# SungFeng-Huang/Meta-TTS

Hardware: AMD Instinct MI355X
Metric: meta-steps/sec (8-task meta-batch, 5 inner steps) (higher is better)
Workload: dtype f32; 1 GPU; C3: Meta-TTS MAML first-order (algorithm=meta_emb_vad, inner=5, meta-batch=8 tasks x (5 support + 5 query utts)), FastSpeech2 base.yaml, outer mean + clip(1.0) + Adam/Noam; meta_batch=8, tasks_per_gpu=8, inner_steps=5, order=first, parallelism=task-dp1, numerics=fp32 MFMA (v_mfma_f32_32x32x2_f32), dropout=on (0.2 / 0.5 / 0.5, counter-based masks), batch_ingestion=inside every timed step (host 12-tuples -> HBM + plans)

## Files before the change

include/mtts.h:

```cpp
#ifndef MTTS_H
#define MTTS_H

#include <stdint.h>

#ifdef __cplusplus
extern "C" {
#endif

typedef struct mtts_handle mtts_handle;

typedef struct mtts_model_cfg {
    int d_model, enc_layers, dec_layers, enc_heads, dec_heads, d_ff, k1, k2;
    int vp_filter, vp_kernel, n_bins, max_seq_len, n_mel, vocab, n_speaker;
    int postnet_dim, postnet_kernel, postnet_layers;
    float pitch_min, pitch_max, energy_min, energy_max;
    int adapt_mask;
    float enc_dropout, dec_dropout, vp_dropout;
    int pitch_frame_level, energy_frame_level;
} mtts_model_cfg;

typedef struct mtts_batch {
    int B, S_max, T_max;
    const int64_t* speakers;
    const int64_t* texts;
// ... 82 lines not shown
int mtts_profile_kinds(void);
const char* mtts_profile_kernel_name(int kind);
int mtts_profile_report(mtts_handle* h, double* out, int kinds);

int mtts_gemm_f32(int form, int M, int N, int K, const float* A, int lda, const float* B, int ldb, float* C, int ldc,
                  const float* bias, float alpha, int flags, int tile, void* hip_stream);
int mtts_gemm_f32_dual(int form, int M, int N, int K, const float* A, int lda, const float* B, int ldb, const float* A2, const float* B2,
                       float* C, int ldc, const float* bias, float alpha, int flags, int tile, void* hip_stream);
int mtts_gemm_bf16(int form, int M, int N, int K, const float* A, int lda, const float* B, int ldb, const float* A2, const float* B2,
                   float* C, int ldc, const float* bias, float alpha, int flags, int tile, void* hip_stream);
int mtts_to_bf16(const float* src, unsigned short* dst, long long n, void* stream);
int mtts_gemm_bf16_planes(int M, int N, int K, const unsigned short* Ah, int lda, const unsigned short* Bh, int ldb, float* C, unsigned short* Ch,
                          int ldc, const float* bias, float alpha, int flags, int tile, void* stream);
long long mtts_plane_problems(mtts_handle* h);
int mtts_xcd_schedule_check(const int* dims, int groups, int cls, int tn, int units_per_group, int* max_load_permille);
int mtts_conv1d_f32(int mode, int L, int Cin, int Cout, int k, const float* x_or_dy, const float* w_or_x, float* out,
                    const float* bias, int tile, void* hip_stream);

int64_t mtts_kernel_ws_bytes(int rows, int n_mat);
int mtts_layernorm_fwd(int rows, int C, const float* a, const float* res, const float* gamma, const float* beta, const unsigned char* mask,
                       float* z, float* y, float* stats, void* ws, void* hip_stream);
int mtts_layernorm_bwd(int rows, int C, const float* dy, const float* z, const float* stats, const float* gamma, const unsigned char* mask,
                       float* dz, float* dgamma, float* dbeta, void* ws, void* hip_stream);
int mtts_softmax_fwd(int n_mat, int L, float* S, void* ws, void* hip_stream);
int mtts_softmax_bwd(int n_mat, int L, const float* P, float* dP, float alpha, void* ws, void* hip_stream);
int mtts_sdpa_fwd(int n_mat, int L, int dk, const float* q, const float* k, const float* v, float* P, float* o, void* ws, void* hip_stream);
int mtts_batchnorm_fwd(int rows, int C, const float* x, const unsigned char* inrect, const float* gamma, const float* beta, int do_tanh,
                       float* stats, float* y, void* ws, void* hip_stream);
int mtts_batchnorm_bwd(int rows, int n_in, int C, const float* dy, const float* y, const float* x, const float* stats, const unsigned char* inrect,
                       const float* gamma, int do_tanh, float* dx, float* dgamma, float* dbeta, void* ws, void* hip_stream);
// ... 140 lines not shown
```

meta_tts_amd/_lib.py:

```python
from __future__ import annotations

import ctypes as C
import os

HERE = os.path.dirname(os.path.abspath(__file__))
DEFAULT_LIB = os.path.join(HERE, "libmtts.so")


class ModelCfg(C.Structure):
    _fields_ = [(n, C.c_int) for n in (
        "d_model", "enc_layers", "dec_layers", "enc_heads", "dec_heads", "d_ff", "k1", "k2",
        "vp_filter", "vp_kernel", "n_bins", "max_seq_len", "n_mel", "vocab", "n_speaker",
        "postnet_dim", "postnet_kernel", "postnet_layers")] + [
        ("pitch_min", C.c_float), ("pitch_max", C.c_float), ("energy_min", C.c_float), ("energy_max", C.c_float),
        ("adapt_mask", C.c_int), ("enc_dropout", C.c_float), ("dec_dropout", C.c_float), ("vp_dropout", C.c_float),
        ("pitch_frame_level", C.c_int), ("energy_frame_level", C.c_int)]


class Batch(C.Structure):
    _fields_ = [("B", C.c_int), ("S_max", C.c_int), ("T_max", C.c_int),
                ("speakers", C.c_void_p), ("texts", C.c_void_p), ("src_lens", C.c_void_p),
                ("mels", C.c_void_p), ("mel_lens", C.c_void_p), ("pitches", C.c_void_p),
                ("energies", C.c_void_p), ("durations", C.c_void_p), ("spk_emb", C.c_void_p)]

# ... 55 lines not shown
    "mtts_sync_pack": (C.c_int, [C.c_void_p, C.c_float]),
    "mtts_sync_unpack": (C.c_int, [C.c_void_p]),
    "mtts_get_synced_losses": (C.c_int, [C.c_void_p, C.c_void_p]),
    "mtts_set_bn_sync": (C.c_int, [C.c_void_p, C.c_int]),
    "mtts_outer_update": (C.c_int, [C.c_void_p, C.c_void_p, C.c_float, C.c_float, C.c_float, C.c_float, C.c_float,
                                    C.c_float, C.c_void_p]),
    "mtts_reset_optimizer": (C.c_int, [C.c_void_p]),
    "mtts_set_grad_accumulation": (C.c_int, [C.c_void_p, C.c_int]),
    "mtts_profile_gemm": (C.c_int, [C.c_void_p, C.c_int]),
    "mtts_profile_kinds": (C.c_int, []),
    "mtts_profile_kernel_name": (C.c_char_p, [C.c_int]),
    "mtts_profile_report": (C.c_int, [C.c_void_p, C.POINTER(C.c_double), C.c_int]),
    "mtts_gemm_f32": (C.c_int, [C.c_int, C.c_int, C.c_int, C.c_int, C.c_void_p, C.c_int, C.c_void_p, C.c_int, C.c_void_p,
                                C.c_int, C.c_void_p, C.c_float, C.c_int, C.c_int, C.c_void_p]),
    "mtts_xcd_schedule_check": (C.c_int, [C.POINTER(C.c_int), C.c_int, C.c_int, C.c_int, C.c_int, C.POINTER(C.c_int)]),
    "mtts_gemm_f32_dual": (C.c_int, [C.c_int, C.c_int, C.c_int, C.c_int, C.c_void_p, C.c_int, C.c_void_p, C.c_int, C.c_void_p, C.c_void_p,
                                     C.c_void_p, C.c_int, C.c_void_p, C.c_float, C.c_int, C.c_int, C.c_void_p]),
    "mtts_to_bf16": (C.c_int, [C.c_void_p, C.c_void_p, C.c_longlong, C.c_void_p]),
    "mtts_gemm_bf16_planes": (C.c_int, [C.c_int, C.c_int, C.c_int, C.c_void_p, C.c_int, C.c_void_p, C.c_int, C.c_void_p, C.c_void_p, C.c_int,
                                        C.c_void_p, C.c_float, C.c_int, C.c_int, C.c_void_p]),
    "mtts_plane_problems": (C.c_longlong, [C.c_void_p]),
    "mtts_gemm_bf16": (C.c_int, [C.c_int, C.c_int, C.c_int, C.c_int, C.c_void_p, C.c_int, C.c_void_p, C.c_int, C.c_void_p, C.c_void_p,
                                 C.c_void_p, C.c_int, C.c_void_p, C.c_float, C.c_int, C.c_int, C.c_void_p]),
    "mtts_conv1d_f32": (C.c_int, [C.c_int, C.c_int, C.c_int, C.c_int, C.c_int, C.c_void_p, C.c_void_p, C.c_void_p,
                                  C.c_void_p, C.c_int, C.c_void_p]),
    "mtts_kernel_ws_bytes": (C.c_int64, [C.c_int, C.c_int]),
    "mtts_layernorm_fwd": (C.c_int, [C.c_int, C.c_int] + [C.c_void_p] * 10),
    "mtts_layernorm_bwd": (C.c_int, [C.c_int, C.c_int] + [C.c_void_p] * 10),
    "mtts_softmax_fwd": (C.c_int, [C.c_int, C.c_int, C.c_void_p, C.c_void_p, C.c_void_p]),
    "mtts_softmax_bwd": (C.c_int, [C.c_int, C.c_int, C.c_void_p, C.c_void_p, C.c_float, C.c_void_p, C.c_void_p]),
# ... 123 lines not shown
```

meta_tts_amd/csrc/gemm.h:

```cpp
#pragma once
#include <algorithm>
#include <cmath>
#include <cstdio>
#include <cstdlib>
#include <vector>

#include "compat.h"
#include "devres.h"
#include "knobs.h"

namespace mtts {

enum GemmForm { GEMM_NT = 0, GEMM_NN = 1, GEMM_TN = 2,
                GEMM_NT_H = 3 };
enum GemmFlags { GEMM_RELU = 1, GEMM_ACCUM = 2, GEMM_LRELU = 4 };

struct GemmGroupDesc {
    long long a_off, b_off, c_off;
    int M, N, K;
    int lda, ldb, ldc;
};

struct XcdSched {
    int on = 0;
// ... 105 lines not shown
    long long colsum_gs = 0;
    const float* colsum_w = nullptr;
    long long colsum_w_gs = 0;
    const float* A2 = nullptr;
    const float* B2 = nullptr;
    long long a2_gs = 0, b2_gs = 0;
    const bf16_t* Ah = nullptr;
    const bf16_t* Bh = nullptr;
    long long bh_gs = 0;
    bf16_t* Ch = nullptr;
    bool plane_only = false;
    LnFuse ln;
    const int* host_dims = nullptr;
    XcdSched xs;
    int wave_prio = 0;
};
inline int gemm_keff(const GemmArgs& g) { return g.A2 ? 2 * g.K : g.K; }


__device__ __forceinline__ int xcd_group_size(int tiles_n, int splitk) {
    const int G = tiles_n * (splitk > 1 ? splitk : 1);
    return G < 64 ? G : 64;
}
__device__ __forceinline__ int xcd_group_remap(int lin, int total, int G) {
    if (G <= 1) return lin;
    const int run = 8 * G, blk = lin / run;
    if ((blk + 1) * run > total) return lin;
    const int r = lin - blk * run;
    return blk * run + (r & 7) * G + (r >> 3);
}
// ... 695 lines not shown
}

template <int BM, int BN, int BK, int KL = 0>
__global__ __launch_bounds__(256) void gemm_f32_multi_dual_kernel(GemmMulti mp) {
    constexpr int F0 = GemmSmem<GEMM_NT, BM, BN, BK>::FLOATS, F1 = GemmSmem<GEMM_NN, BM, BN, BK>::FLOATS, F2 = GemmSmem<GEMM_TN, BM, BN, BK>::FLOATS;
    constexpr int FL = F0 > F1 ? (F0 > F2 ? F0 : F2) : (F1 > F2 ? F1 : F2);
    __shared__ __attribute__((aligned(16))) float smem[FL];
    int p, z, bx;
    if (!gemm_multi_locate(mp, p, z, bx)) return;
    const int form = mp.form[p];
    if (form == GEMM_NT) gemm_f32_body<GEMM_NT, BM, BN, BK, true, 2, 2, 0, true, KL>(mp.g[p], z, bx, smem);
    else if (form == GEMM_NN) gemm_f32_body<GEMM_NN, BM, BN, BK, true, 2, 2, 0, true, KL>(mp.g[p], z, bx, smem);
    else gemm_f32_body<GEMM_TN, BM, BN, BK, true, 2, 2, 0, true, KL>(mp.g[p], z, bx, smem);
}

enum GemmKind {
    GK_F32_64_BK16 = 0,
    GK_F32_64_BK32 = 3,
    GK_F32_128 = 6,
    GK_GLDS = 9,
    GK_MULTI16 = 12, GK_MULTI32 = 13, GK_GLDS_MULTI = 14, GK_OTHER = 15,
    GK_MULTI16_DUAL = 16, GK_MULTI32_DUAL = 17, GK_GLDS_MULTI_DUAL = 18,
    GK_BF16_64 = 19,
    GK_BF16_128 = 22,
    GK_BF16_MULTI64 = 25, GK_BF16_MULTI128 = 26, GK_BF16_MULTI64_DUAL = 27, GK_BF16_MULTI128_DUAL = 28,
    GK_ATTN_FWD = 29,
    GK_BF16_64_H64 = 30, GK_BF16_64_H32 = 31, GK_BF16_128_H = 32,
    GK_BF16_MULTI64_PLANES = 33,
    GK_COUNT = 34
};
inline const char* gemm_kind_name(int k) {
    static const char* names[GK_COUNT] = {
        "gemm_f32_kernel<0, 64, 64, 16, true, 2, 2, 0, 4>", "gemm_f32_kernel<1, 64, 64, 16, true, 2, 2, 0, 4>", "gemm_f32_kernel<2, 64, 64, 16, true, 2, 2, 0, 4>",
        "gemm_f32_kernel<0, 64, 64, 32, true, 2, 2, 0, 4>", "gemm_f32_kernel<1, 64, 64, 32, true, 2, 2, 0, 4>", "gemm_f32_kernel<2, 64, 64, 32, true, 2, 2, 0, 4>",
        "gemm_f32_kernel<0, 128, 128, ...>", "gemm_f32_kernel<1, 128, 128, ...>", "gemm_f32_kernel<2, 128, 128, ...>",
        "gemm_glds_kernel<0>", "gemm_glds_kernel<1>", "gemm_glds_kernel<2>",
        "gemm_f32_multi_kernel<64, 64, 16, 4>", "gemm_f32_multi_kernel<64, 64, 32, 4>", "gemm_glds_multi_kernel",
        "gemm_f32_kernel<other>", "gemm_f32_multi_dual_kernel<64, 64, 16, 4>", "gemm_f32_multi_dual_kernel<64, 64, 32, 4>", "gemm_glds_multi_dual_kernel",
        "gemm_bf16_kernel<0, 64, 64, 32, 1>", "gemm_bf16_kernel<1, 64, 64, 32, 1>", "gemm_bf16_kernel<2, 64, 64, 32, 1>",
        "gemm_bf16_kernel<0, 128, 128, 32, 1>", "gemm_bf16_kernel<1, 128, 128, 32, 1>", "gemm_bf16_kernel<2, 128, 128, 32, 1>",
        "gemm_bf16_multi_kernel<64, 64, 32, 1, false>", "gemm_bf16_multi_kernel<128, 128, 32, 1, false>",
        "gemm_bf16_multi_kernel<64, 64, 32, 1, true>", "gemm_bf16_multi_kernel<128, 128, 32, 1, true>", "attn_fwd_kernel",
        "gemm_bf16_kernel<3, 64, 64, 64, 1>", "gemm_bf16_kernel<3, 64, 64, 32, 1>", "gemm_bf16_kernel<3, 128, 128, 32, 1>",
        "gemm_bf16_multi_planes_kernel<64, 64, 32, 64, 1>"};
    return (k >= 0 && k < GK_COUNT) ? names[k] : "?";
}

struct GemmProfiler {
    struct Rec { int kernel; double flops; hipEvent_t e0, e1; int form = 0, tile = 0, N = 0, K = 0, groups = 0, splitk = 1; double rows = 0, bytes = 0; int tag = 0; };
    int ctx = 0;
    int tag = 0;
    std::vector<Rec> recs;
    std::vector<hipEvent_t> pool;
    size_t used = 0;
    bool enabled = false;
    hipEvent_t get(DevHeap& heap) {
        if (used == pool.size()) { hipEvent_t e = nullptr; heap.event(e); pool.push_back(e); }
        return pool[used++];
    }
// ... 18 lines not shown
inline int gemm_kloop_variant() { return knobs().kloop; }
inline int gemm_kloop_for(const GemmArgs& g, int bk) {
    const bool ok = (g.taps <= 1 || g.tap_k % bk == 0) && (g.a_tap_k >= 0x40000000 || g.a_tap_k % bk == 0);
    return ok ? gemm_kloop_variant() : 0;
}
inline int gemm_xcd_swizzle() { return kGemmXcdSwizzle; }
inline int gemm_default_bk() { return kGemmDefaultBk; }
inline bool gemm_default_pipe() { return kGemmDefaultPipe; }

struct GemmWorkspace { float* ws = nullptr; int* ctr = nullptr; };
constexpr long long kSplitWsFloats = 16ll << 20;
constexpr int kSplitCtrs = 1 << 16;
constexpr int kLnCtrs = 4096;

struct GemmPending { int form; GemmArgs g; int max_M, max_N, groups; double flops, rows, bytes; };
struct GemmBatch { bool open = false; std::vector<GemmPending> q; int force_family = 0; int force_tile = 0; };

struct GemmCtx {
    GemmBatch batch;
    GemmProfiler prof;
    GemmWorkspace wsp;
    int last_kind = GK_OTHER;
    long long plane_problems = 0;
    bool bf16 = false;
    const char* error = nullptr;
    bool flushing = false;
    bool prefer_bk16 = false;
    int wave_prio = 0;
    bool no_glds = false;
    DevHeap* heap = nullptr;
    int alloc_workspace(DevHeap& h) {
// ... 31 lines not shown
inline bool gemm_use_glds() { return gemm_glds_mode() != 0; }
inline bool gemm_glds_ok(const GemmArgs& g) { return !(g.taps > 1 && g.tap_k % 32 != 0); }
inline int gemm_tiles_n(const GemmArgs& g, int max_N, int t) { return (max_N + t - 1) / t + (g.colsum ? 1 : 0); }
inline long gemm_glds_max_wgs() { return 768L; }
#if !defined(MTTS_EMU)
inline void gemm_glds_launch(int form, const GemmArgs& g, dim3 grid, hipStream_t stream);
inline void gemm_glds_multi_launch(const GemmMulti& mp, dim3 grid, hipStream_t stream, bool dual = false);
#endif

inline bool gemm_bf16_ok(const GemmArgs& g);
inline bool gemm_bf16_planes_ok(int form, const GemmArgs& g);
inline int gemm_bf16_launch(int form, const GemmArgs& g, int T, dim3 grid, hipStream_t stream, int pf);
inline int gemm_bf16_multi_launch(const GemmMulti& mp, int T, bool dual, dim3 grid, hipStream_t stream);
inline int gemm_bf16_tile(double rows, int tiles_n128) { return std::ceil(rows / 128.0) * tiles_n128 >= 512.0 ? 128 : 64; }

inline bool gemm_xcd_sched_for(GemmArgs& g, int max_M, int max_N, int groups, int S, int tile) {
    g.xs.on = 0;
    if (!knobs().xcd_sched || (groups != 8 && groups != 4 && groups != 2) || groups < knobs().xcd_sched_min_groups || !g.host_dims || !g.dimptr || g.table || S != 1) return false;
    int dims[8] = {0};
    for (int z = 0; z < groups; ++z) dims[z] = g.host_dims[z] * g.dim_mult;
    const int tn = gemm_tiles_n(g, max_N, tile);
    if (g.dim_sel == 0) xcd_sched_build(g.xs, dims, 1, tn, 0, tile, groups);
    else xcd_sched_build(g.xs, dims, 2, 1, ((max_M + tile - 1) / tile) * tn, 64, groups);
    if (g.xs.maxlen <= 0) g.xs.on = 0;
    if (knobs().xcd_sched_debug && g.xs.on) fprintf(stderr, "xcd_sched cls %d tn %d maxlen %d pool %d\n", g.xs.on, g.xs.tn, g.xs.maxlen, g.xs.P[8]);
    return g.xs.on != 0;
}
inline long gemm_xcd_sched_slots(const XcdSched& s) { return 8L * s.maxlen * (s.on == 1 ? s.tn : 1); }
inline bool gemm_panel_order_for(const GemmArgs& g, int form, double rows, int max_M, int max_N, int groups) {
    if (!knobs().panel_order || g.table || groups >= 8 || groups < 1) return false;
    if (std::ceil(rows / 64.0) * gemm_tiles_n(g, max_N, 64) > (double)gemm_glds_max_wgs()) return false;
    const double K = (double)gemm_keff(g);
    const double a_bytes = form == GEMM_TN ? rows * max_M : rows / groups * (g.lda > 0 ? g.lda : K);
    const double b_bytes = form == GEMM_TN ? rows * max_N : (double)max_N * K;
    (void)max_M;
    return b_bytes > a_bytes;
}

inline void gemm_launch(GemmCtx& cx, int form, const GemmArgs& g_in, int max_M, int max_N, int groups, hipStream_t stream,
                        int tile = 0, double alg_flops = 0.0, long long total_M = 0, double alg_bytes = 0.0) {
    if (max_M <= 0 || max_N <= 0 || groups <= 0) return;
    GemmArgs g = g_in;
    g.swizzle = gemm_xcd_swizzle();
    g.wave_prio = cx.wave_prio;
    if (!(cx.bf16 && gemm_bf16_ok(g) && gemm_bf16_planes_ok(form, g))) {
        if (g.plane_only) { cx.error = "plane-only GEMM problem outside the bf16 plane path"; return; }
        g.Ah = g.Bh = nullptr;
    }
    if (!cx.bf16) g.Ch = nullptr;
    const int user_tile = tile;
    const double rows = total_M > 0 ? (double)total_M : (double)max_M * groups;
// ... 24 lines not shown
    bool pipe = gemm_default_pipe();
    int bk = gemm_default_bk();
    bool glds = false;
    const bool bf16 = cx.bf16 && gemm_bf16_ok(g) && !g.A2;
    if (bf16 && user_tile == 0) tile = gemm_bf16_tile(rows, gemm_tiles_n(g, max_N, 128));
#if !defined(MTTS_EMU)
    if (bf16) { if (tile == 4064) tile = 64; }
    else if (tile == 4064) { glds = gemm_glds_ok(g); tile = 64; }
    else if (user_tile == 0 && tile == 64) {
        const long wgs = (long)std::ceil(rows / 64.0) * gemm_tiles_n(g, max_N, 64);
        glds = gemm_use_glds() && gemm_glds_ok(g) && wgs <= gemm_glds_max_wgs() && !cx.no_glds && !g.ln.y;
    }
#else
    if (tile == 4064) tile = 64;
#endif
    const int ablate = tile / 10000;
    tile %= 10000;
    if (tile >= 1000) { pipe = (tile / 1000) & 1; bk = (tile / 2000) ? 32 : 16; tile %= 1000; }
    if (user_tile == 0 && !g.table && gemm_keff(g) >= 1024 && (form == GEMM_NT || form == GEMM_TN)) bk = 32;
    if (g.taps > 1 && g.tap_k % 32 != 0) bk = 16;
    if (bf16) bk = 32;
    const int S = 1;
    { int used = 0; if (!gemm_ln_bind(cx, form, g, max_M, groups, bf16 ? 0 : tile, used)) return; }
    const int nth = 256;
    const long grid_tiles = ntiles(tile);
    dim3 block(nth), grid((unsigned)(grid_tiles * S), 1, (unsigned)groups);
    if (gemm_xcd_sched_for(g, max_M, max_N, groups, S, tile)) grid = dim3((unsigned)gemm_xcd_sched_slots(g.xs), 1, 1);
    else if (gemm_panel_order_for(g, form, rows, max_M, max_N, groups)) {
        g.swizzle = 2; g.po_tiles_m = (max_M + tile - 1) / tile;
        grid = dim3((unsigned)xcd_panel_slots(g.po_tiles_m, gemm_tiles_n(g, max_N, tile), S), 1, (unsigned)groups);
    }
    GemmProfiler& prof = cx.prof;
    hipEvent_t e0 = nullptr, e1 = nullptr;
    if (prof.enabled) { e0 = prof.get(*cx.heap); e1 = prof.get(*cx.heap); hipEventRecord(e0, stream); }
    int kind = GK_OTHER;
#define MTTS_GEMM_CASE(F, T)                                                                              \
    if (form == F && tile == T) {                                                                         \
        if (pipe && T == 64) {                                                                            \
            const int kl = gemm_kloop_for(g, bk);                                                         \
            if (F == GEMM_NT && g.ln.ctr) {       \
                if (bk == 32) MTTS_LAUNCH((gemm_f32_kernel<GEMM_NT, 64, 64, 32, true, 2, 2, 0, 4, true>), grid, block, stream, g);   \
                else MTTS_LAUNCH((gemm_f32_kernel<GEMM_NT, 64, 64, 16, true, 2, 2, 0, 4, true>), grid, block, stream, g);            \
// ... 12 lines not shown
        else if (bk == 32 && pipe) { MTTS_LAUNCH((gemm_f32_kernel<F, T, T, 32, true>), grid, block, stream, g); kind = (T == 64 ? GK_F32_64_BK32 : GK_F32_128) + F; }   \
        else if (bk == 32) { MTTS_LAUNCH((gemm_f32_kernel<F, T, T, 32, false>), grid, block, stream, g); kind = T == 64 ? GK_OTHER : GK_F32_128 + F; }     \
        else if (pipe) { MTTS_LAUNCH((gemm_f32_kernel<F, T, T, 16, true>), grid, block, stream, g); kind = (T == 64 ? GK_F32_64_BK16 : GK_F32_128) + F; }          \
        else { MTTS_LAUNCH((gemm_f32_kernel<F, T, T, 16, false>), grid, block, stream, g); kind = T == 64 ? GK_OTHER : GK_F32_128 + F; }                   \
    }
    if (bf16) {
        if (g.Ah) ++cx.plane_problems;
        kind = gemm_bf16_launch(form, g, tile, grid, stream, (user_tile % 10000) / 1000);
    } else
#if !defined(MTTS_EMU)
    if (glds) {
        gemm_glds_launch(form, g, grid, stream);
        kind = GK_GLDS + form;
    } else
#endif
    {
#if defined(MTTS_GEMM_ABLATION)
#define MTTS_ABL(A) if (ablate == A && form == GEMM_NT) { MTTS_LAUNCH((gemm_f32_kernel<GEMM_NT, 64, 64, 16, true, 2, 2, A>), grid, block, stream, g); return; }
        MTTS_ABL(1) MTTS_ABL(2) MTTS_ABL(3) MTTS_ABL(4) MTTS_ABL(7) MTTS_ABL(8) MTTS_ABL(15) MTTS_ABL(6) MTTS_ABL(14)
#undef MTTS_ABL
#else
        (void)ablate;
#endif
        MTTS_GEMM_CASE(GEMM_NT, 128) MTTS_GEMM_CASE(GEMM_NT, 64)
        MTTS_GEMM_CASE(GEMM_NN, 128) MTTS_GEMM_CASE(GEMM_NN, 64)
        MTTS_GEMM_CASE(GEMM_TN, 128) MTTS_GEMM_CASE(GEMM_TN, 64)
    }
#undef MTTS_GEMM_CASE
    cx.last_kind = kind;
    if (prof.enabled) {
        hipEventRecord(e1, stream);
        GemmProfiler::Rec rec{kind, alg_flops, e0, e1};
        rec.form = form; rec.tile = bf16 ? 16000 + tile : (glds ? 4064 : tile); rec.N = max_N; rec.K = gemm_keff(g); rec.groups = groups; rec.splitk = S;
        rec.rows = rows;
        rec.bytes = alg_bytes; rec.tag = prof.tag;
        prof.recs.push_back(rec);
    }
}

inline bool batch_full_regime(const std::vector<GemmPending>& q) {
    double wgs = 0.0;
    for (const GemmPending& p : q) wgs += std::ceil(p.rows / 64.0) * gemm_tiles_n(p.g, p.max_N, 64);
    return wgs > (double)gemm_glds_max_wgs();
}
inline void gemm_batch_end(GemmCtx& cx, hipStream_t stream) {
    GemmBatch& b = cx.batch;
    b.open = false;
    if (b.q.empty()) return;
// ... 80 lines not shown
        max_groups = std::max(max_groups, p.groups);
        flops += p.flops; rows += p.rows; bytes += p.bytes;
    }
    hipEvent_t e0 = nullptr, e1 = nullptr;
    if (prof.enabled) { e0 = prof.get(*cx.heap); e1 = prof.get(*cx.heap); hipEventRecord(e0, stream); }
    dim3 block(256), grid((unsigned)mp.start[mp.n], 1, 1);
    bool bk32 = true;
    int maxK = 0;
    for (int i = 0; i < mp.n; ++i) {
        if (mp.g[i].taps > 1 && mp.g[i].tap_k % 32 != 0) bk32 = false;
        maxK = std::max(maxK, gemm_keff(mp.g[i]));
    }
    bool glds = gemm_use_glds() && small_batch && !cx.no_glds && ln_used == 0;
    if (b.force_family) { glds = b.force_family == 4064; bk32 = bk32 && b.force_family == 32; if (bk32) maxK = std::max(maxK, 1024); }
    for (int i = 0; i < mp.n; ++i) glds = glds && gemm_glds_ok(mp.g[i]);
    int kind = GK_MULTI16;
    if (bf16) {
        for (int i = 0; i < mp.n; ++i) if (mp.g[i].Ah) ++cx.plane_problems;
        kind = gemm_bf16_multi_launch(mp, T, any_dual, grid, stream);
        glds = false;
    } else
#if !defined(MTTS_EMU)
    if (glds) { gemm_glds_multi_launch(mp, grid, stream, any_dual); kind = any_dual ? GK_GLDS_MULTI_DUAL : GK_GLDS_MULTI; }
    else
#endif
    if (bk32 && maxK >= 1024 && !cx.prefer_bk16) {
        int kl = gemm_kloop_variant();
        for (int i = 0; i < mp.n; ++i) kl = std::min(kl, gemm_kloop_for(mp.g[i], 32));
        if (any_dual) {
            if (kl == 4) MTTS_LAUNCH((gemm_f32_multi_dual_kernel<64, 64, 32, 4>), grid, block, stream, mp);
            else if (kl == 1) MTTS_LAUNCH((gemm_f32_multi_dual_kernel<64, 64, 32, 1>), grid, block, stream, mp);
            else MTTS_LAUNCH((gemm_f32_multi_dual_kernel<64, 64, 32, 0>), grid, block, stream, mp);
            kind = GK_MULTI32_DUAL;
        } else {
            if (ln_used > 0) MTTS_LAUNCH((gemm_f32_multi_kernel<64, 64, 32, 4, true>), grid, block, stream, mp);
            else if (kl == 4) MTTS_LAUNCH((gemm_f32_multi_kernel<64, 64, 32, 4>), grid, block, stream, mp);
            else if (kl == 1) MTTS_LAUNCH((gemm_f32_multi_kernel<64, 64, 32, 1>), grid, block, stream, mp);
            else MTTS_LAUNCH((gemm_f32_multi_kernel<64, 64, 32, 0>), grid, block, stream, mp);
            kind = GK_MULTI32;
        }
    } else {
// ... 1 lines not shown
        for (int i = 0; i < mp.n; ++i) kl = std::min(kl, gemm_kloop_for(mp.g[i], 16) == 4 ? 4 : 0);
        if (any_dual) {
            if (kl == 4) MTTS_LAUNCH((gemm_f32_multi_dual_kernel<64, 64, 16, 4>), grid, block, stream, mp);
            else MTTS_LAUNCH((gemm_f32_multi_dual_kernel<64, 64, 16, 0>), grid, block, stream, mp);
            kind = GK_MULTI16_DUAL;
        } else {
            if (ln_used > 0) MTTS_LAUNCH((gemm_f32_multi_kernel<64, 64, 16, 4, true>), grid, block, stream, mp);
            else if (kl == 4) MTTS_LAUNCH((gemm_f32_multi_kernel<64, 64, 16, 4>), grid, block, stream, mp);
            else MTTS_LAUNCH((gemm_f32_multi_kernel<64, 64, 16, 0>), grid, block, stream, mp);
        }
    }
    cx.last_kind = kind;
    if (prof.enabled) {
        hipEventRecord(e1, stream);
        GemmProfiler::Rec rec{kind, flops, e0, e1};
        rec.form = 3; rec.tile = bf16 ? 16000 + T : (glds ? 4064 : 64); rec.N = mp.n; rec.K = maxK; rec.groups = mp.start[mp.n]; rec.splitk = max_split; rec.rows = rows; rec.bytes = bytes; rec.tag = prof.tag;
        prof.recs.push_back(rec);
    }
    b.q.clear();
}

}
```

meta_tts_amd/csrc/knobs.h:

```cpp
#pragma once
#include <cstdlib>

namespace mtts {

struct Knobs {
    int kloop = 4;
    int glds = 0;
    int xcd_sched = 1;
    int xcd_sched_min_groups = 8;
    int xcd_sched_debug = 0;
    int panel_order = 1;
    int single_multi = 1;
    int batch_splitk = 1;
    int defer_wgrad = 1;
    int side_pred_all = 1;
    int pred_side = 1;
    int pred_early = 1;
    int pred_batch = 1;
    int enc_ahead = 1;
    int enc_ahead_all = 1;
    int enc_ahead_query = 1;
    int upd_overlap = 1;
    int ln_fold_side = 1;
    int side_bk16 = 1;
    int main_prio = 1;
    int fused_attn = 1;
    int attn_sort = 1;
    int ln_fuse = 0;
    int so_keep_act = 1;
    int so_keep_grad = 1;
    int so_defer_post = 1;
    int so_fuse_drop = 1;
    int so_ln_part = 1;
    int so_pred_side = 1;
    int so_table_side = 1;
    int ablate_ln = 0;
    int attn_diag_mask = 0;
};

inline Knobs read_knobs() {
    Knobs k;
    const struct { const char* name; int* v; } table[] = {
        {"MTTS_KLOOP", &k.kloop}, {"MTTS_GLDS", &k.glds}, {"MTTS_XCD_SCHED", &k.xcd_sched}, {"MTTS_XCD_SCHED_MIN_GROUPS", &k.xcd_sched_min_groups},
        {"MTTS_PANEL_ORDER", &k.panel_order}, {"MTTS_SINGLE_MULTI", &k.single_multi}, {"MTTS_BATCH_SPLITK", &k.batch_splitk},
        {"MTTS_DEFER_WGRAD", &k.defer_wgrad}, {"MTTS_SIDE_PRED_ALL", &k.side_pred_all}, {"MTTS_PRED_SIDE", &k.pred_side}, {"MTTS_PRED_EARLY", &k.pred_early},
        {"MTTS_PRED_BATCH", &k.pred_batch}, {"MTTS_ENC_AHEAD", &k.enc_ahead}, {"MTTS_ENC_AHEAD_ALL", &k.enc_ahead_all}, {"MTTS_ENC_AHEAD_QUERY", &k.enc_ahead_query},
        {"MTTS_UPD_OVERLAP", &k.upd_overlap}, {"MTTS_LN_FOLD_SIDE", &k.ln_fold_side}, {"MTTS_SIDE_BK16", &k.side_bk16}, {"MTTS_MAIN_PRIO", &k.main_prio},
        {"MTTS_FUSED_ATTN", &k.fused_attn}, {"MTTS_ATTN_SORT", &k.attn_sort}, {"MTTS_LN_FUSE", &k.ln_fuse}, {"MTTS_SO_KEEP_ACT", &k.so_keep_act},
        {"MTTS_SO_KEEP_GRAD", &k.so_keep_grad}, {"MTTS_SO_DEFER_POST", &k.so_defer_post}, {"MTTS_SO_FUSE_DROP", &k.so_fuse_drop}, {"MTTS_SO_LN_PART", &k.so_ln_part},
        {"MTTS_SO_PRED_SIDE", &k.so_pred_side}, {"MTTS_SO_TABLE_SIDE", &k.so_table_side},
#if defined(MTTS_ABLATE)
        {"MTTS_ABLATE_LN", &k.ablate_ln},
#endif
#if defined(MTTS_ATTN_DIAG)
        {"MTTS_ATTN_DIAG_MASK", &k.attn_diag_mask},
#endif
    };
    for (const auto& t : table)
        if (const char* e = getenv(t.name)) *t.v = atoi(e);
    if (k.kloop != 0 && k.kloop != 1 && k.kloop != 4) k.kloop = 4;
    k.glds = k.glds != 0;
    k.xcd_sched_debug = getenv("MTTS_XCD_SCHED_DEBUG") != nullptr;
    return k;
}
inline const Knobs& knobs() {
    static const Knobs k = read_knobs();
    return k;
}

}
```

meta_tts_amd/csrc/mtts.hip:

```cpp
#include "../../include/mtts.h"

#include "comm.h"
#include "engine.h"
#include "vocoder.h"
#include "dvector.h"
#include "melfront.h"
#include "griffin.h"
#include "preprocess.h"
#include "resample.h"
#include "pitch.h"
#include "vad.h"
#include "speakereval.h"
#include "tsne.h"
#include "dtw.h"

using namespace mtts;

static int copy_losses_impl(Engine& e, const float* dev, float* host, int n);
static int copy_losses(Engine& e, const float* dev, float* host, int n) { return copy_losses_impl(e, dev, host, n); }

struct mtts_handle {
    Engine eng;
    Comm comm;
    float* sup_losses_dev = nullptr;
// ... 464 lines not shown
        for (int k = 0; k < GK_COUNT; ++k) for (int j = 0; j < 4; ++j) out[k * 4 + j] += r[k][j];
    }
    return 0;
}

static GemmCtx& kernel_ctx() {
    static thread_local GemmCtx cx;
    return cx;
}
static int kernel_launch_rc() {
    GemmCtx& cx = kernel_ctx();
    if (cx.error) { cx.error = nullptr; (void)hipGetLastError(); return -1; }
    return hipGetLastError() == hipSuccess ? 0 : -1;
}
static bool tile_code_ok(int tile) {
    return tile == 0 || tile == 4064 || ((tile % 1000 == 64 || tile % 1000 == 128) && tile % 10000 < 4000);
}

int mtts_gemm_f32(int form, int M, int N, int K, const float* A, int lda, const float* B, int ldb, float* C, int ldc,
                  const float* bias, float alpha, int flags, int tile, void* stream) {
    if (form < 0 || form > 2 || !tile_code_ok(tile)) return -1;
    GemmArgs g;
    g.A = A; g.B = B; g.C = C; g.lda = lda; g.ldb = ldb; g.ldc = ldc; g.M = M; g.N = N; g.K = K;
    g.bias = bias; g.alpha = alpha; g.flags = flags & 0xff;
    if (flags & ~0xff) return -1;
    gemm_launch(kernel_ctx(), form, g, M, N, 1, (hipStream_t)stream, tile);
    return kernel_launch_rc();
}

int mtts_xcd_schedule_check(const int* dims_in, int groups, int cls, int tn, int units_per_group, int* max_load_permille) {
    if (!dims_in || (groups != 8 && groups != 4 && groups != 2) || (cls != 1 && cls != 2) || tn < 1) return -1;
// ... 11 lines not shown
    const long slots = gemm_xcd_sched_slots(s);
    for (long lin = 0; lin < slots; ++lin) {
        int z = -1, tile = -1;
        if (!xcd_sched_locate(s, (int)lin, z, tile)) continue;
        if (z < 0 || z >= groups || tile < 0 || tile >= (int)seen[z].size() || seen[z][tile]++) return -1;
        work[lin & 7] += cls == 1 ? 1 : std::max(dims[z], 1);
    }
    for (int z = 0; z < groups; ++z)
        for (int v : seen[z]) if (v != 1) return -1;
    if (max_load_permille) {
        long long mx = 0;
        for (int x = 0; x < 8; ++x) mx = std::max(mx, work[x]);
        *max_load_permille = total > 0 ? (int)(mx * 8000 / total) : 0;
    }
    return (int)slots;
}

int mtts_gemm_f32_dual(int form, int M, int N, int K, const float* A, int lda, const float* B, int ldb, const float* A2, const float* B2,
                       float* C, int ldc, const float* bias, float alpha, int flags, int tile, void* stream) {
    if (form < 0 || form > 2 || !tile_code_ok(tile) || !A2 || !B2 || (flags & ~0xff)) return -1;
    GemmArgs g;
    g.A = A; g.B = B; g.A2 = A2; g.B2 = B2; g.C = C; g.lda = lda; g.ldb = ldb; g.ldc = ldc; g.M = M; g.N = N; g.K = K;
    g.bias = bias; g.alpha = alpha; g.flags = flags & 0xff;
    gemm_launch(kernel_ctx(), form, g, M, N, 1, (hipStream_t)stream, tile);
    return kernel_launch_rc();
}

int mtts_gemm_bf16(int form, int M, int N, int K, const float* A, int lda, const float* B, int ldb, const float* A2, const float* B2,
                   float* C, int ldc, const float* bias, float alpha, int flags, int tile, void* stream) {
    if (form < 0 || form > 2 || (tile != 0 && ((tile % 1000 != 64 && tile % 1000 != 128) || tile / 1000 > 4)) || (flags & ~0xff) || ((A2 == nullptr) != (B2 == nullptr))) return -1;
// ... 312 lines not shown
```

Measured before the change: 6.287 meta-steps/s.

## Add mixed 128/64 tile GEMM kernels for large fp32 MFMA problems

Adds a mixed-tile fp32 GEMM path. The full 128-row blocks of each problem are covered by 128x128 tiles, and the ragged tail plus the column-sum tiles use 64x64 tiles, inside one launch for both single and batched multi-GEMM calls. With the default knob (mode 1), it applies to large NT problems with K>=1024 whose work-group count exceeds a threshold, with the number of big tiles budgeted in multiples of 512. The aim is more data reuse per tile and fewer work-groups on big GEMMs while keeping fine granularity at the edges. The cost is more kernel variants, shared memory sized for 128x128 on every block, and possible load imbalance from mixing tile sizes. Test entry points for tile coverage and a paired GEMM are also added.

```diff
diff --git a/include/mtts.h b/include/mtts.h
--- a/include/mtts.h
+++ b/include/mtts.h
@@ -120,6 +120,9 @@
                           int ldc, const float* bias, float alpha, int flags, int tile, void* stream);
 long long mtts_plane_problems(mtts_handle* h);
 int mtts_xcd_schedule_check(const int* dims, int groups, int cls, int tn, int units_per_group, int* max_load_permille);
+int mtts_mixed_tiles_check(const int* rows, int groups, int N, int has_cs, int cap, int* big_tiles);
+int mtts_gemm_pair_f32(int tile, const float* dy, const float* w, float* dx, const int* rows_dev, const int* rowmap, int groups, int max_M, int N, int K,
+                       const float* a, const float* b, float* c, float* colsum, const float* colsum_w, int R, int M2, int N2, void* stream);
 int mtts_conv1d_f32(int mode, int L, int Cin, int Cout, int k, const float* x_or_dy, const float* w_or_x, float* out,
                     const float* bias, int tile, void* hip_stream);
 
diff --git a/meta_tts_amd/_lib.py b/meta_tts_amd/_lib.py
--- a/meta_tts_amd/_lib.py
+++ b/meta_tts_amd/_lib.py
@@ -93,6 +93,9 @@
     "mtts_gemm_f32": (C.c_int, [C.c_int, C.c_int, C.c_int, C.c_int, C.c_void_p, C.c_int, C.c_void_p, C.c_int, C.c_void_p,
                                 C.c_int, C.c_void_p, C.c_float, C.c_int, C.c_int, C.c_void_p]),
     "mtts_xcd_schedule_check": (C.c_int, [C.POINTER(C.c_int), C.c_int, C.c_int, C.c_int, C.c_int, C.POINTER(C.c_int)]),
+    "mtts_mixed_tiles_check": (C.c_int, [C.POINTER(C.c_int), C.c_int, C.c_int, C.c_int, C.c_int, C.POINTER(C.c_int)]),
+    "mtts_gemm_pair_f32": (C.c_int, [C.c_int, C.c_void_p, C.c_void_p, C.c_void_p, C.c_void_p, C.c_void_p, C.c_int, C.c_int, C.c_int, C.c_int,
+                                     C.c_void_p, C.c_void_p, C.c_void_p, C.c_void_p, C.c_void_p, C.c_int, C.c_int, C.c_int, C.c_void_p]),
     "mtts_gemm_f32_dual": (C.c_int, [C.c_int, C.c_int, C.c_int, C.c_int, C.c_void_p, C.c_int, C.c_void_p, C.c_int, C.c_void_p, C.c_void_p,
                                      C.c_void_p, C.c_int, C.c_void_p, C.c_float, C.c_int, C.c_int, C.c_void_p]),
     "mtts_to_bf16": (C.c_int, [C.c_void_p, C.c_void_p, C.c_longlong, C.c_void_p]),
diff --git a/meta_tts_amd/csrc/gemm.h b/meta_tts_amd/csrc/gemm.h
--- a/meta_tts_amd/csrc/gemm.h
+++ b/meta_tts_amd/csrc/gemm.h
@@ -143,6 +143,7 @@
     const int* host_dims = nullptr;
     XcdSched xs;
     int wave_prio = 0;
+    int m_split = 0;
 };
 inline int gemm_keff(const GemmArgs& g) { return g.A2 ? 2 * g.K : g.K; }
 
@@ -868,6 +869,77 @@
     else gemm_f32_body<GEMM_TN, BM, BN, BK, true, 2, 2, 0, true, KL>(mp.g[p], z, bx, smem);
 }
 
+struct MixedTile { int big, m0, n0, cs; };
+__host__ __device__ __forceinline__ int gemm_mixed_split(int M, int cap) {
+    const int whole = M > 0 ? (M / 128) * 128 : 0;
+    return whole < cap ? whole : cap;
+}
+__host__ __device__ __forceinline__ bool gemm_mixed_locate(int M, int N, int has_cs, int cap, int t, MixedTile& o) {
+    if (M <= 0 || N <= 0 || t < 0) return false;
+    const int split = gemm_mixed_split(M, cap);
+    const int tn128 = (N + 127) / 128, tnc = (N + 63) / 64, tn64 = tnc + (has_cs ? 1 : 0);
+    const int nbig = (split / 128) * tn128;
+    if (t < nbig) { o.big = 1; o.m0 = (t / tn128) * 128; o.n0 = (t % tn128) * 128; o.cs = 0; return true; }
+    t -= nbig;
+    const int ncs = has_cs ? split / 64 : 0;
+    if (t < ncs) { o.big = 0; o.m0 = t * 64; o.n0 = tnc * 64; o.cs = 1; return true; }
+    t -= ncs;
+    const int tail_m = (M - split + 63) / 64;
+    if (t >= tail_m * tn64) return false;
+    const int mi = t / tn64, ni = t - mi * tn64;
+    o.big = 0; o.m0 = split + mi * 64; o.n0 = ni * 64; o.cs = (has_cs && ni == tnc) ? 1 : 0;
+    return true;
+}
+__host__ __device__ __forceinline__ int gemm_mixed_slots_of(int M, int N, int has_cs, int cap) {
+    if (M <= 0 || N <= 0) return 0;
+    const int split = gemm_mixed_split(M, cap);
+    return (split / 128) * ((N + 127) / 128) + (has_cs ? split / 64 : 0) + ((M - split + 63) / 64) * ((N + 63) / 64 + (has_cs ? 1 : 0));
+}
+inline int gemm_mixed_slots(int max_M, int N, int has_cs, int cap) {
+    int best = gemm_mixed_slots_of(max_M, N, has_cs, cap);
+    for (int m = 127; m < max_M; m += 128) best = std::max(best, gemm_mixed_slots_of(m, N, has_cs, cap));
+    return best;
+}
+
+template <int FORM, int BM, int BN, int KL>
+__device__ __forceinline__ void gemm_f32_mixed_tile(const GemmArgs& g, const GemmProb& pr, int z, int m0, int n0, bool cs_tile, float* smem) {
+    constexpr int TM = (BM / 2) / 32, TN = (BN / 2) / 32;
+    f32x16 acc[TM][TN];
+#pragma unroll
+    for (int i = 0; i < TM; ++i)
+#pragma unroll
+        for (int j = 0; j < TN; ++j)
+#pragma unroll
+            for (int r = 0; r < 16; ++r) acc[i][j][r] = 0.f;
+    gemm_f32_kloop<FORM, BM, BN, 32, true, 2, 2, 0, KL>(g, pr, z, m0, n0, cs_tile, 0, (pr.K + 31) / 32, smem, acc);
+    gemm_finish<TM, TN, 2, 2>(g, pr, z, m0, n0, cs_tile, acc);
+}
+template <int FORM, int KL>
+__device__ __forceinline__ void gemm_f32_mixed_body(const GemmArgs& g, int z, int t, float* smem) {
+    if (g.wave_prio > 0) MTTS_SETPRIO_HIGH();
+    const GemmProb pr = gemm_resolve(g, z);
+    if (pr.K <= 0) return;
+    MixedTile mt;
+    if (!gemm_mixed_locate(pr.M, pr.N, gemm_has_colsum<FORM>(g) ? 1 : 0, g.m_split, t, mt)) return;
+    if (mt.big) gemm_f32_mixed_tile<FORM, 128, 128, KL>(g, pr, z, mt.m0, mt.n0, false, smem);
+    else gemm_f32_mixed_tile<FORM, 64, 64, KL>(g, pr, z, mt.m0, mt.n0, mt.cs != 0, smem);
+}
+template <int FORM, int KL = 4>
+__global__ __launch_bounds__(256) void gemm_f32_mixed_kernel(GemmArgs g) {
+    __shared__ __attribute__((aligned(16))) float smem[GemmSmem<FORM, 128, 128, 32>::FLOATS];
+    gemm_f32_mixed_body<FORM, KL>(g, (int)blockIdx.z, (int)blockIdx.x, smem);
+}
+template <int KL = 4>
+__global__ __launch_bounds__(256) void gemm_f32_multi_mixed_kernel(GemmMulti mp) {
+    __shared__ __attribute__((aligned(16))) float smem[GemmSmem<GEMM_NT, 128, 128, 32>::FLOATS];
+    int p, z, bx;
+    if (!gemm_multi_locate(mp, p, z, bx)) return;
+    const int form = mp.form[p];
+    if (form == GEMM_NT) gemm_f32_mixed_body<GEMM_NT, KL>(mp.g[p], z, bx, smem);
+    else if (form == GEMM_NN) gemm_f32_mixed_body<GEMM_NN, KL>(mp.g[p], z, bx, smem);
+    else gemm_f32_mixed_body<GEMM_TN, KL>(mp.g[p], z, bx, smem);
+}
+
 enum GemmKind {
     GK_F32_64_BK16 = 0,
     GK_F32_64_BK32 = 3,
@@ -881,7 +953,9 @@
     GK_ATTN_FWD = 29,
     GK_BF16_64_H64 = 30, GK_BF16_64_H32 = 31, GK_BF16_128_H = 32,
     GK_BF16_MULTI64_PLANES = 33,
-    GK_COUNT = 34
+    GK_F32_MIXED = 34,
+    GK_MULTI_MIXED = 37,
+    GK_COUNT = 38
 };
 inline const char* gemm_kind_name(int k) {
     static const char* names[GK_COUNT] = {
@@ -896,7 +970,8 @@
         "gemm_bf16_multi_kernel<64, 64, 32, 1, false>", "gemm_bf16_multi_kernel<128, 128, 32, 1, false>",
         "gemm_bf16_multi_kernel<64, 64, 32, 1, true>", "gemm_bf16_multi_kernel<128, 128, 32, 1, true>", "attn_fwd_kernel",
         "gemm_bf16_kernel<3, 64, 64, 64, 1>", "gemm_bf16_kernel<3, 64, 64, 32, 1>", "gemm_bf16_kernel<3, 128, 128, 32, 1>",
-        "gemm_bf16_multi_planes_kernel<64, 64, 32, 64, 1>"};
+        "gemm_bf16_multi_planes_kernel<64, 64, 32, 64, 1>",
+        "gemm_f32_mixed_kernel<0, 4>", "gemm_f32_mixed_kernel<1, 4>", "gemm_f32_mixed_kernel<2, 4>", "gemm_f32_multi_mixed_kernel<4>"};
     return (k >= 0 && k < GK_COUNT) ? names[k] : "?";
 }
 
@@ -945,7 +1020,7 @@
 constexpr int kLnCtrs = 4096;
 
 struct GemmPending { int form; GemmArgs g; int max_M, max_N, groups; double flops, rows, bytes; };
-struct GemmBatch { bool open = false; std::vector<GemmPending> q; int force_family = 0; int force_tile = 0; };
+struct GemmBatch { bool open = false; std::vector<GemmPending> q; int force_family = 0; int force_tile = 0; bool force_mixed = false; };
 
 struct GemmCtx {
     GemmBatch batch;
@@ -1007,9 +1082,12 @@
 inline int gemm_bf16_multi_launch(const GemmMulti& mp, int T, bool dual, dim3 grid, hipStream_t stream);
 inline int gemm_bf16_tile(double rows, int tiles_n128) { return std::ceil(rows / 128.0) * tiles_n128 >= 512.0 ? 128 : 64; }
 
+inline bool gemm_xcd_sched_applies(const GemmArgs& g, int groups, int S) {
+    return knobs().xcd_sched && (groups == 8 || groups == 4 || groups == 2) && groups >= knobs().xcd_sched_min_groups && g.host_dims && g.dimptr && !g.table && S == 1;
+}
 inline bool gemm_xcd_sched_for(GemmArgs& g, int max_M, int max_N, int groups, int S, int tile) {
     g.xs.on = 0;
-    if (!knobs().xcd_sched || (groups != 8 && groups != 4 && groups != 2) || groups < knobs().xcd_sched_min_groups || !g.host_dims || !g.dimptr || g.table || S != 1) return false;
+    if (!gemm_xcd_sched_applies(g, groups, S)) return false;
     int dims[8] = {0};
     for (int z = 0; z < groups; ++z) dims[z] = g.host_dims[z] * g.dim_mult;
     const int tn = gemm_tiles_n(g, max_N, tile);
@@ -1028,6 +1106,18 @@
     const double b_bytes = form == GEMM_TN ? rows * max_N : (double)max_N * K;
     (void)max_M;
     return b_bytes > a_bytes;
+}
+
+inline bool gemm_mixed_ok(const GemmCtx& cx, const GemmArgs& g, int max_N) {
+    return !cx.bf16 && !g.A2 && !g.table && !g.ln.y && !g.plane_only && g.N == max_N && gemm_kloop_variant() == 4 && gemm_kloop_for(g, 32) == 4;
+}
+constexpr int kMixedRound = 512;
+inline int gemm_mixed_rule(int max_M, int max_N, int groups, long& budget) {
+    const int tn128 = (max_N + 127) / 128;
+    const long per_mtile = (long)tn128 * groups;
+    const long mt = std::min<long>(max_M / 128, budget / per_mtile);
+    budget -= mt * per_mtile;
+    return (int)mt * 128;
 }
 
 inline void gemm_launch(GemmCtx& cx, int form, const GemmArgs& g_in, int max_M, int max_N, int groups, hipStream_t stream,
@@ -1082,18 +1172,37 @@
 #else
     if (tile == 4064) tile = 64;
 #endif
+    const bool mixed_code = user_tile % 10000 == 3192;
+    if (mixed_code) tile -= 128;
     const int ablate = tile / 10000;
     tile %= 10000;
     if (tile >= 1000) { pipe = (tile / 1000) & 1; bk = (tile / 2000) ? 32 : 16; tile %= 1000; }
     if (user_tile == 0 && !g.table && gemm_keff(g) >= 1024 && (form == GEMM_NT || form == GEMM_TN)) bk = 32;
     if (g.taps > 1 && g.tap_k % 32 != 0) bk = 16;
     if (bf16) bk = 32;
+    int m_split = 0;
+    if (!bf16 && !glds && tile == 64 && pipe && gemm_mixed_ok(cx, g, max_N)) {
+        const int mode = user_tile == 0 ? knobs().mixed_tiles : 0;
+        if ((mixed_code && bk == 32) || mode == 2) { bk = 32; m_split = (max_M / 128) * 128; }
+        else if (mode == 1 && bk == 32 && form == GEMM_NT && !gemm_xcd_sched_applies(g, groups, 1)) {
+            const long wgs = (long)std::ceil(rows / 64.0) * gemm_tiles_n(g, max_N, 64);
+            if (wgs > gemm_glds_max_wgs()) {
+                const long all = (long)(max_M / 128) * ((max_N + 127) / 128) * groups;
+                long budget = all / kMixedRound * kMixedRound;
+                m_split = gemm_mixed_rule(max_M, max_N, groups, budget);
+            }
+        }
+    }
     const int S = 1;
     { int used = 0; if (!gemm_ln_bind(cx, form, g, max_M, groups, bf16 ? 0 : tile, used)) return; }
     const int nth = 256;
     const long grid_tiles = ntiles(tile);
     dim3 block(nth), grid((unsigned)(grid_tiles * S), 1, (unsigned)groups);
-    if (gemm_xcd_sched_for(g, max_M, max_N, groups, S, tile)) grid = dim3((unsigned)gemm_xcd_sched_slots(g.xs), 1, 1);
+    if (m_split > 0) {
+        g.m_split = m_split; g.swizzle = 0; g.xs.on = 0;
+        grid = dim3((unsigned)gemm_mixed_slots(max_M, max_N, g.colsum ? 1 : 0, m_split), 1, (unsigned)groups);
+    }
+    else if (gemm_xcd_sched_for(g, max_M, max_N, groups, S, tile)) grid = dim3((unsigned)gemm_xcd_sched_slots(g.xs), 1, 1);
     else if (gemm_panel_order_for(g, form, rows, max_M, max_N, groups)) {
         g.swizzle = 2; g.po_tiles_m = (max_M + tile - 1) / tile;
         grid = dim3((unsigned)xcd_panel_slots(g.po_tiles_m, gemm_tiles_n(g, max_N, tile), S), 1, (unsigned)groups);
@@ -1136,6 +1245,12 @@
         kind = GK_GLDS + form;
     } else
 #endif
+    if (m_split > 0) {
+        if (form == GEMM_NT) MTTS_LAUNCH((gemm_f32_mixed_kernel<GEMM_NT, 4>), grid, block, stream, g);
+        else if (form == GEMM_NN) MTTS_LAUNCH((gemm_f32_mixed_kernel<GEMM_NN, 4>), grid, block, stream, g);
+        else MTTS_LAUNCH((gemm_f32_mixed_kernel<GEMM_TN, 4>), grid, block, stream, g);
+        kind = GK_F32_MIXED + form;
+    } else
     {
 #if defined(MTTS_GEMM_ABLATION)
 #define MTTS_ABL(A) if (ablate == A && form == GEMM_NT) { MTTS_LAUNCH((gemm_f32_kernel<GEMM_NT, 64, 64, 16, true, 2, 2, A>), grid, block, stream, g); return; }
@@ -1153,7 +1268,7 @@
     if (prof.enabled) {
         hipEventRecord(e1, stream);
         GemmProfiler::Rec rec{kind, alg_flops, e0, e1};
-        rec.form = form; rec.tile = bf16 ? 16000 + tile : (glds ? 4064 : tile); rec.N = max_N; rec.K = gemm_keff(g); rec.groups = groups; rec.splitk = S;
+        rec.form = form; rec.tile = bf16 ? 16000 + tile : (glds ? 4064 : (m_split > 0 ? 192 : tile)); rec.N = max_N; rec.K = gemm_keff(g); rec.groups = groups; rec.splitk = S;
         rec.rows = rows;
         rec.bytes = alg_bytes; rec.tag = prof.tag;
         prof.recs.push_back(rec);
@@ -1264,6 +1379,38 @@
     bool glds = gemm_use_glds() && small_batch && !cx.no_glds && ln_used == 0;
     if (b.force_family) { glds = b.force_family == 4064; bk32 = bk32 && b.force_family == 32; if (bk32) maxK = std::max(maxK, 1024); }
     for (int i = 0; i < mp.n; ++i) glds = glds && gemm_glds_ok(mp.g[i]);
+    bool mixed = false;
+    {
+        const int mode = b.force_family ? (b.force_mixed && b.force_family == 32 ? 2 : 0) : knobs().mixed_tiles;
+        bool fam = mode != 0 && !bf16 && !glds && !any_dual && ln_used == 0 && max_split == 1 && bk32 && !cx.prefer_bk16 && gemm_kloop_variant() == 4;
+        if (mode == 1) fam = fam && maxK >= 1024 && !small_batch;
+        for (int i = 0; i < mp.n && fam; ++i) fam = gemm_kloop_for(mp.g[i], 32) == 4;
+        if (fam) {
+            int split[kGemmMultiMax] = {0};
+            long budget = 0;
+            auto can = [&](int i) { return gemm_mixed_ok(cx, mp.g[i], b.q[i].max_N) && !(mode == 1 && (mp.g[i].xs.on || mp.form[i] != GEMM_NT)); };
+            for (int i = 0; i < mp.n; ++i)
+                if (can(i)) budget += (long)(b.q[i].max_M / 128) * ((b.q[i].max_N + 127) / 128) * b.q[i].groups;
+            budget = budget / kMixedRound * kMixedRound;
+            for (int i = 0; i < mp.n; ++i) {
+                if (!can(i)) continue;
+                split[i] = mode == 2 ? (b.q[i].max_M / 128) * 128 : gemm_mixed_rule(b.q[i].max_M, b.q[i].max_N, b.q[i].groups, budget);
+                mixed = mixed || split[i] > 0;
+            }
+            if (mixed) {
+                for (int i = 0; i < mp.n; ++i) {
+                    long slots = mp.start[i + 1] - mp.start[i];
+                    if (split[i] > 0) {
+                        mp.g[i].m_split = split[i]; mp.g[i].xs.on = 0; mp.xcd_group[i] = 0;
+                        mp.tiles_pg[i] = gemm_mixed_slots(b.q[i].max_M, b.q[i].max_N, mp.g[i].colsum ? 1 : 0, split[i]);
+                        slots = (long)mp.tiles_pg[i] * b.q[i].groups;
+                    }
+                    mp.start[i + 1] = mp.start[i] + (int)((slots + 7) & ~7L);
+                }
+                grid = dim3((unsigned)mp.start[mp.n], 1, 1);
+            }
+        }
+    }
     int kind = GK_MULTI16;
     if (bf16) {
         for (int i = 0; i < mp.n; ++i) if (mp.g[i].Ah) ++cx.plane_problems;
@@ -1274,7 +1421,8 @@
     if (glds) { gemm_glds_multi_launch(mp, grid, stream, any_dual); kind = any_dual ? GK_GLDS_MULTI_DUAL : GK_GLDS_MULTI; }
     else
 #endif
-    if (bk32 && maxK >= 1024 && !cx.prefer_bk16) {
+    if (mixed) { MTTS_LAUNCH((gemm_f32_multi_mixed_kernel<4>), grid, block, stream, mp); kind = GK_MULTI_MIXED; }
+    else if (bk32 && maxK >= 1024 && !cx.prefer_bk16) {
         int kl = gemm_kloop_variant();
         for (int i = 0; i < mp.n; ++i) kl = std::min(kl, gemm_kloop_for(mp.g[i], 32));
         if (any_dual) {
@@ -1306,7 +1454,7 @@
     if (prof.enabled) {
         hipEventRecord(e1, stream);
         GemmProfiler::Rec rec{kind, flops, e0, e1};
-        rec.form = 3; rec.tile = bf16 ? 16000 + T : (glds ? 4064 : 64); rec.N = mp.n; rec.K = maxK; rec.groups = mp.start[mp.n]; rec.splitk = max_split; rec.rows = rows; rec.bytes = bytes; rec.tag = prof.tag;
+        rec.form = 3; rec.tile = bf16 ? 16000 + T : (glds ? 4064 : (mixed ? 192 : 64)); rec.N = mp.n; rec.K = maxK; rec.groups = mp.start[mp.n]; rec.splitk = max_split; rec.rows = rows; rec.bytes = bytes; rec.tag = prof.tag;
         prof.recs.push_back(rec);
     }
     b.q.clear();
diff --git a/meta_tts_amd/csrc/knobs.h b/meta_tts_amd/csrc/knobs.h
--- a/meta_tts_amd/csrc/knobs.h
+++ b/meta_tts_amd/csrc/knobs.h
@@ -26,6 +26,7 @@
     int main_prio = 1;
     int fused_attn = 1;
     int attn_sort = 1;
+    int mixed_tiles = 1;
     int ln_fuse = 0;
     int so_keep_act = 1;
     int so_keep_grad = 1;
@@ -46,7 +47,7 @@
         {"MTTS_DEFER_WGRAD", &k.defer_wgrad}, {"MTTS_SIDE_PRED_ALL", &k.side_pred_all}, {"MTTS_PRED_SIDE", &k.pred_side}, {"MTTS_PRED_EARLY", &k.pred_early},
         {"MTTS_PRED_BATCH", &k.pred_batch}, {"MTTS_ENC_AHEAD", &k.enc_ahead}, {"MTTS_ENC_AHEAD_ALL", &k.enc_ahead_all}, {"MTTS_ENC_AHEAD_QUERY", &k.enc_ahead_query},
         {"MTTS_UPD_OVERLAP", &k.upd_overlap}, {"MTTS_LN_FOLD_SIDE", &k.ln_fold_side}, {"MTTS_SIDE_BK16", &k.side_bk16}, {"MTTS_MAIN_PRIO", &k.main_prio},
-        {"MTTS_FUSED_ATTN", &k.fused_attn}, {"MTTS_ATTN_SORT", &k.attn_sort}, {"MTTS_LN_FUSE", &k.ln_fuse}, {"MTTS_SO_KEEP_ACT", &k.so_keep_act},
+        {"MTTS_FUSED_ATTN", &k.fused_attn}, {"MTTS_ATTN_SORT", &k.attn_sort}, {"MTTS_LN_FUSE", &k.ln_fuse}, {"MTTS_MIXED_TILES", &k.mixed_tiles}, {"MTTS_SO_KEEP_ACT", &k.so_keep_act},
         {"MTTS_SO_KEEP_GRAD", &k.so_keep_grad}, {"MTTS_SO_DEFER_POST", &k.so_defer_post}, {"MTTS_SO_FUSE_DROP", &k.so_fuse_drop}, {"MTTS_SO_LN_PART", &k.so_ln_part},
         {"MTTS_SO_PRED_SIDE", &k.so_pred_side}, {"MTTS_SO_TABLE_SIDE", &k.so_table_side},
 #if defined(MTTS_ABLATE)
@@ -59,6 +60,7 @@
     for (const auto& t : table)
         if (const char* e = getenv(t.name)) *t.v = atoi(e);
     if (k.kloop != 0 && k.kloop != 1 && k.kloop != 4) k.kloop = 4;
+    if (k.mixed_tiles < 0 || k.mixed_tiles > 2) k.mixed_tiles = 1;
     k.glds = k.glds != 0;
     k.xcd_sched_debug = getenv("MTTS_XCD_SCHED_DEBUG") != nullptr;
     return k;
diff --git a/meta_tts_amd/csrc/mtts.hip b/meta_tts_amd/csrc/mtts.hip
--- a/meta_tts_amd/csrc/mtts.hip
+++ b/meta_tts_amd/csrc/mtts.hip
@@ -502,7 +502,7 @@
     return hipGetLastError() == hipSuccess ? 0 : -1;
 }
 static bool tile_code_ok(int tile) {
-    return tile == 0 || tile == 4064 || ((tile % 1000 == 64 || tile % 1000 == 128) && tile % 10000 < 4000);
+    return tile == 0 || tile == 4064 || tile == 3192 || ((tile % 1000 == 64 || tile % 1000 == 128) && tile % 10000 < 4000);
 }
 
 int mtts_gemm_f32(int form, int M, int N, int K, const float* A, int lda, const float* B, int ldb, float* C, int ldc,
@@ -544,6 +544,61 @@
         *max_load_permille = total > 0 ? (int)(mx * 8000 / total) : 0;
     }
     return (int)slots;
+}
+
+int mtts_mixed_tiles_check(const int* rows, int groups, int N, int has_cs, int cap, int* big_tiles) {
+    if (!rows || groups < 1 || N < 1 || cap < 0 || cap % 128 != 0) return -1;
+    int max_M = 0;
+    for (int z = 0; z < groups; ++z) max_M = std::max(max_M, rows[z]);
+    const int slots = gemm_mixed_slots(max_M, N, has_cs ? 1 : 0, cap);
+    const int tnc = (N + 63) / 64, tn = tnc + (has_cs ? 1 : 0);
+    long long nbig = 0;
+    for (int z = 0; z < groups; ++z) {
+        const int M = rows[z], tm = M > 0 ? (M + 63) / 64 : 0;
+        std::vector<int> seen((size_t)tm * tn, 0);
+        bool small_seen = false;
+        for (int t = 0; t < slots; ++t) {
+            MixedTile mt;
+            if (!gemm_mixed_locate(M, N, has_cs ? 1 : 0, cap, t, mt)) continue;
+            const int sz = mt.big ? 128 : 64;
+            if (mt.m0 < 0 || mt.n0 < 0 || mt.m0 % sz || mt.n0 % sz || mt.m0 >= M) return -1;
+            if (mt.big) {
+                if (small_seen || mt.cs || mt.m0 + 128 > M || mt.m0 + 128 > cap || mt.n0 >= N) return -1;
+                ++nbig;
+                for (int i = 0; i < 2; ++i)
+                    for (int j = 0; j < 2; ++j) {
+                        const int mi = mt.m0 / 64 + i, ni = mt.n0 / 64 + j;
+                        if (ni < tnc && seen[(size_t)mi * tn + ni]++) return -1;
+                    }
+            } else {
+                small_seen = true;
+                const int mi = mt.m0 / 64, ni = mt.n0 / 64;
+                if (ni >= tn || (mt.cs != 0) != (has_cs && ni == tnc)) return -1;
+                if (seen[(size_t)mi * tn + ni]++) return -1;
+            }
+        }
+        for (int v : seen) if (v != 1) return -1;
+    }
+    if (big_tiles) *big_tiles = (int)nbig;
+    return slots;
+}
+
+int mtts_gemm_pair_f32(int tile, const float* dy, const float* w, float* dx, const int* rows_dev, const int* rowmap, int groups, int max_M, int N, int K,
+                       const float* a, const float* b, float* c, float* colsum, const float* colsum_w, int R, int M2, int N2, void* stream) {
+    if (!tile_code_ok(tile) || tile == 0 || tile == 4064 || tile % 10000 < 2000 || groups < 1 || !dy || !w || !dx || !rows_dev || !a || !b || !c) return -1;
+    GemmCtx& cx = kernel_ctx();
+    GemmArgs g1;
+    g1.A = a; g1.lda = M2; g1.B = b; g1.ldb = N2; g1.C = c; g1.ldc = N2; g1.M = M2; g1.N = N2; g1.K = R;
+    g1.colsum = colsum; g1.colsum_w = colsum ? colsum_w : nullptr;
+    GemmArgs g2;
+    g2.A = dy; g2.lda = K; g2.a_gs = (long long)max_M * K; g2.B = w; g2.ldb = N; g2.b_gs = (long long)K * N; g2.C = dx; g2.ldc = N; g2.c_gs = (long long)max_M * N;
+    g2.M = max_M; g2.N = N; g2.K = K; g2.dimptr = rows_dev; g2.c_rowmap = rowmap; g2.c_rowmap_gs = max_M;
+    cx.batch.force_family = 32; cx.batch.force_tile = 64; cx.batch.force_mixed = tile % 10000 == 3192;
+    cx.batch.q.push_back(GemmPending{GEMM_TN, g1, M2, N2, 1, 0.0, (double)M2, 0.0});
+    cx.batch.q.push_back(GemmPending{GEMM_NN, g2, max_M, N, groups, 0.0, (double)max_M * groups, 0.0});
+    gemm_batch_end(cx, (hipStream_t)stream);
+    cx.batch.force_family = 0; cx.batch.force_tile = 0; cx.batch.force_mixed = false;
+    return kernel_launch_rc();
 }
 
 int mtts_gemm_f32_dual(int form, int M, int N, int K, const float* A, int lda, const float* B, int ldb, const float* A2, const float* B2,
```

Result: no change. 6.273 meta-steps/s (-0.2%).
